# XuanchenLi/Topo4D

Measured on AMD Instinct MI355X. Metric: rasterizer fwd+bwd views/sec, higher is better.
Workload: dtype f32; 1 GPU; C2: 24 views x 512x512, P=30000 vertex-bound Gaussians, precomputed RGB, opacity scenario A, forward+backward, per-view gradients; frames=64, steps_per_rank=20, parallelism=frame-sharded x1, frames_per_launch=1, sync_mode=lazy (capacity learned by checked warm-up), frames_in_flight=3

## Files before the change

topo4d_amd/csrc/t4d_raster.hip:

```cpp
#include "t4d_raster_plan.h"

#include <hip/hip_runtime.h>
#include <stdint.h>
#include <stdio.h>
#include <string.h>
#include <vector>

#include "t4d_activations.h"
#include "t4d_tile_div.h"
#include "t4d_raster_visit_pad.h"

#define T4D_EXPORT extern "C" __attribute__((visibility("default")))

namespace {

#ifndef T4D_BWD_BATCH
#define T4D_BWD_BATCH 128
#endif
constexpr int kBwdBatch = T4D_BWD_BATCH;
constexpr int kRankSortMax = 512;
constexpr int kHist = 1024;
constexpr int kBuckets = 24;
constexpr int kGP = T4D_GRAD_PAIR_FLOATS;
constexpr int kSnapFloats = 6;

thread_local char g_err[512] = "";

enum KernelId { K_PREPROCESS = 0, K_SCAN_TILES, K_SCATTER, K_SORT_TILES, K_RENDER_FWD, K_RENDER_BWD, K_PREPROCESS_BWD,
                K_SORT_LONG, K_FWD_LONG, K_RENDER_BWD_LONG, K_COUNT };
const char *const kKernelNames[K_COUNT] = { "k_preprocess", "k_scan_tiles", "k_scatter", "k_sort_tiles", "k_render_fwd",
                                            "k_render_bwd", "k_preprocess_bwd", "k_sort_long", "k_fwd_long", "k_render_bwd_long" };
struct ProfRec { int id; hipEvent_t a, b; };
bool g_prof_on = false;
std::vector<ProfRec> g_prof;

struct Layout {
    size_t status, view_total, view_cursor, tile_count, bucket_fill, slot_tab, zero_end;
    size_t snap, live;
    size_t tile_off, chunk_sum, order, items, xy, depth, conic_opacity, rgb, clamped, pair_off, pair_rank, keys, sort_tmp, final_T, n_contrib, total;
};

struct DevStatus {
    uint32_t overflow;
    uint32_t max_pairs;
    unsigned long long total_pairs;
    uint32_t max_tile_pairs;
    uint32_t grid_sync;
    uint32_t live_segments;
};

inline size_t align_up(size_t x, size_t a = 256) { return (x + a - 1) / a * a; }

Layout make_layout(const T4DProblem &p)
{
    Layout L;
    const size_t V = (size_t)p.n_views, P = (size_t)p.P;
    const size_t T = (size_t)tile_dims(p.W, p.H).T;
    const size_t HW = (size_t)p.H * p.W;
    const size_t cap = (size_t)p.pair_capacity;
    size_t o = 0;
    L.status = o;        o = align_up(o + sizeof(DevStatus));
    L.view_total = o;    o = align_up(o + V * 4);
    L.view_cursor = o;   o = align_up(o + V * kCursorSegs * 4);
    L.tile_count = o;    o = align_up(o + V * T * 4);
    L.bucket_fill = o;   o = align_up(o + kBuckets * 4);
    const size_t slots = seg_mode(p) != 0 ? V * seg_slots_per_view(p, T) : 0;
    L.slot_tab = o;      o = align_up(o + slots * 16);
    L.zero_end = o;
    L.snap = o;          o = align_up(o + slots * kSnapFloats * kBlock * 4);
    L.live = o;          o = align_up(o + (seg_mode(p) == 2 ? slots * 4 : 0));
    L.tile_off = o;      o = align_up(o + V * T * 4);
    L.chunk_sum = o;     o = align_up(o + V * ((T + kScanChunk - 1) / kScanChunk) * 4);
    L.order = o;         o = align_up(o + (size_t)kBuckets * V * T * 4);
    L.items = o;         o = align_up(o + V * T * 16);
    L.xy = o;            o = align_up(o + V * P * 8);
    L.depth = o;         o = align_up(o + V * P * 4);
    L.conic_opacity = o; o = align_up(o + V * P * 16);
    L.rgb = o;           o = align_up(o + (p.sh_coeffs > 0 ? V * P * 12 : 0));
    L.clamped = o;       o = align_up(o + (p.sh_coeffs > 0 ? V * P : 0));
    L.pair_off = o;      o = align_up(o + V * P * 4);
    L.pair_rank = o;     o = align_up(o + V * cap * 4);
    L.keys = o;          o = align_up(o + V * cap * 8);
    L.sort_tmp = o;      o = align_up(o + V * cap * 8);
    L.final_T = o;       o = align_up(o + V * HW * 4);
    L.n_contrib = o;     o = align_up(o + V * HW * 4);
    L.total = o;
    return L;
}

struct KP {
    int V, P, H, W, gx, gy, T, deg, M;
    float scale_modifier;
    uint32_t cap;
    uint32_t nseg, seg_cap;
    uint32_t seg_shift;
    const float *views, *means3D, *opacities, *scales, *rotations, *cov3D_precomp, *colors_precomp, *shs;
    DevStatus *status;
    uint32_t *view_total, *view_cursor, *tile_count, *bucket_fill, *tile_off, *chunk_sum, *order, *pair_off, *pair_rank;
    int n_chunks;
    int long_bins_elsewhere;
    int raw_params;
    uint4 *items;
    float2 *xy;
    float *depth;
    float4 *conic_opacity;
    float *rgb;
    uint8_t *clamped;
    unsigned long long *keys, *sort_tmp;
    float *cut_r2;
    float *final_T;
    uint32_t *n_contrib;
    float *out_color, *out_depth, *out_alpha;
    int32_t *radii;
    const float *dL_dcolor, *dL_ddepth, *dL_dalpha;
    float *grad_pair;
    float *dL_dmeans3D, *dL_dmeans2D, *dL_dcolors, *dL_dshs, *dL_dopacities, *dL_dscales, *dL_drotations, *dL_dcov3D;
    float *tile_dot;
    float *cotangent_dot;
    uint32_t tile_blocks;
    uint32_t fill_blocks;
    uint32_t fill_vec;
    uint4 *slot_tab;
    float *snap;
    uint32_t slots_per_view;
    uint32_t fused_sort;
    unsigned long long *host_status;
    uint32_t seg_min_pairs;
    uint32_t *live;
    uint32_t slots_by_offset;
    uint32_t views_per_set;
    T4DDiv div_gx;
    T4DDiv div_gy;
    T4DDiv div_spans;
    T4DDiv div_blocks;
    uint32_t div_blocks_ok;
    uint32_t div_ok;
};

typedef const __attribute__((address_space(4))) KP *kp_kernarg_p;
__device__ __forceinline__ kp_kernarg_p kernarg_kp()
{
    kp_kernarg_p p = (kp_kernarg_p)__builtin_amdgcn_kernarg_segment_ptr();
    asm volatile("" : "+s"(p));
    return p;
}

__device__ __forceinline__ float ndc2pix(float v, int S)
{
#pragma clang fp contract(off)
    return ((v + 1.0f) * S - 1.0f) * 0.5f;
}

__device__ __forceinline__ void tile_rect(float px, float py, int r, int gx, int gy, int &x0, int &y0, int &x1, int &y1)
{
    x0 = min(gx, max(0, (int)((px - r) / T4D_TILE_X)));
    y0 = min(gy, max(0, (int)((py - r) / T4D_TILE_Y)));
    x1 = min(gx, max(0, (int)((px + r + T4D_TILE_X - 1) / T4D_TILE_X)));
    y1 = min(gy, max(0, (int)((py + r + T4D_TILE_Y - 1) / T4D_TILE_Y)));
}

typedef const __attribute__((address_space(4))) float *const_float_p;
struct ViewRecord {
    float view[16], proj[16], campos[3], bg[3], tanx, tany;
};
__device__ __forceinline__ ViewRecord load_view_record(const float *views, const int v)
{
    const_float_p p = (const_float_p)(views + (size_t)v * T4D_VIEW_FLOATS);
    ViewRecord r;
#pragma unroll
    for (int i = 0; i < 16; i++) { r.view[i] = p[i]; r.proj[i] = p[16 + i]; }
#pragma unroll
    for (int i = 0; i < 3; i++) { r.campos[i] = p[32 + i]; r.bg[i] = p[35 + i]; }
    r.tanx = p[38]; r.tany = p[39];
    return r;
}

__device__ __forceinline__ size_t param_row0(const KP &kp, const int v)
{
    return kp.views_per_set ? (size_t)((uint32_t)v / kp.views_per_set) * (size_t)kp.P : (size_t)0;
}

__device__ __forceinline__ uint32_t seg_slot0(const KP &kp, const uint32_t off, const uint32_t tile)
{
    static_assert((kSegLongMin & (kSegLongMin - 1)) == 0, "a shift");
    return (off >> kp.seg_shift) + (kp.slots_by_offset ? off / (uint32_t)kSegLongMin : tile);
}

__device__ __forceinline__ uint32_t wave_incl_scan(uint32_t v)
{
    const int lane = threadIdx.x & 63;
#pragma unroll
    for (int d = 1; d < 64; d <<= 1) {
        uint32_t o = __shfl_up(v, d, 64);
        if (lane >= d) v += o;
    }
    return v;
}

template <int CTRL, int ROW_MASK = 0xf, int BANK_MASK = 0xf>
__device__ __forceinline__ float dpp0(float v)
{
    return __int_as_float(__builtin_amdgcn_update_dpp(0, __float_as_int(v), CTRL, ROW_MASK, BANK_MASK, false));
}

__device__ __forceinline__ float wave_sum_to_lane63(float v)
{
    v += dpp0<0xB1>(v);
    v += dpp0<0x4E>(v);
    v += dpp0<0x141>(v);
    v += dpp0<0x140>(v);
    v += dpp0<0x142, 0xA>(v);
    v += dpp0<0x143, 0xC>(v);
    return v;
}

__device__ __forceinline__ void quat_rot(const float4 q, float R[9])
{
#pragma clang fp contract(off)
    const float r = q.x, x = q.y, y = q.z, z = q.w;
    R[0] = 1.f - 2.f * (y * y + z * z); R[1] = 2.f * (x * y - r * z);       R[2] = 2.f * (x * z + r * y);
    R[3] = 2.f * (x * y + r * z);       R[4] = 1.f - 2.f * (x * x + z * z); R[5] = 2.f * (y * z - r * x);
    R[6] = 2.f * (x * z - r * y);       R[7] = 2.f * (y * z + r * x);       R[8] = 1.f - 2.f * (x * x + y * y);
}

__device__ __forceinline__ void cov3d_from_scale_rot(const float *scale, float mod, const float4 q, float cov[6])
{
#pragma clang fp contract(off)
    float R[9], M[9];
    quat_rot(q, R);
    const float s[3] = { mod * scale[0], mod * scale[1], mod * scale[2] };
#pragma unroll
    for (int i = 0; i < 3; i++)
#pragma unroll
        for (int k = 0; k < 3; k++) M[i * 3 + k] = R[i * 3 + k] * s[k];
    cov[0] = M[0] * M[0] + M[1] * M[1] + M[2] * M[2];
    cov[1] = M[0] * M[3] + M[1] * M[4] + M[2] * M[5];
    cov[2] = M[0] * M[6] + M[1] * M[7] + M[2] * M[8];
    cov[3] = M[3] * M[3] + M[4] * M[4] + M[5] * M[5];
    cov[4] = M[3] * M[6] + M[4] * M[7] + M[5] * M[8];
    cov[5] = M[6] * M[6] + M[7] * M[7] + M[8] * M[8];
}

__device__ __forceinline__ void ewa_rows(const float *mean, const float *view, float fx, float fy, float tanx, float tany,
                                         float T0[3], float T1[3], float t[3], bool &inx, bool &iny)
{
#pragma clang fp contract(off)
    t[0] = view[0] * mean[0] + view[4] * mean[1] + view[8] * mean[2] + view[12];
    t[1] = view[1] * mean[0] + view[5] * mean[1] + view[9] * mean[2] + view[13];
    t[2] = view[2] * mean[0] + view[6] * mean[1] + view[10] * mean[2] + view[14];
    const float limx = T4D_FRUSTUM_CLAMP * tanx, limy = T4D_FRUSTUM_CLAMP * tany;
    const float txtz = t[0] / t[2], tytz = t[1] / t[2];
    inx = !(txtz < -limx || txtz > limx);
    iny = !(tytz < -limy || tytz > limy);
    t[0] = fminf(limx, fmaxf(-limx, txtz)) * t[2];
    t[1] = fminf(limy, fmaxf(-limy, tytz)) * t[2];
    const float J00 = fx / t[2], J02 = -(fx * t[0]) / (t[2] * t[2]);
    const float J11 = fy / t[2], J12 = -(fy * t[1]) / (t[2] * t[2]);
#pragma unroll
    for (int j = 0; j < 3; j++) {
        T0[j] = J00 * view[j * 4 + 0] + J02 * view[j * 4 + 2];
        T1[j] = J11 * view[j * 4 + 1] + J12 * view[j * 4 + 2];
    }
}

__device__ __forceinline__ void sym3_mul(const float c[6], const float v[3], float o[3])
{
#pragma clang fp contract(off)
    o[0] = c[0] * v[0] + c[1] * v[1] + c[2] * v[2];
    o[1] = c[1] * v[0] + c[3] * v[1] + c[4] * v[2];
    o[2] = c[2] * v[0] + c[4] * v[1] + c[5] * v[2];
}

__device__ __forceinline__ void sh_basis(int deg, const float d[3], float b[16])
{
#pragma clang fp contract(off)
    const float x = d[0], y = d[1], z = d[2];
    b[0] = T4D_SH_C0;
    if (deg > 0) {
        b[1] = -T4D_SH_C1 * y; b[2] = T4D_SH_C1 * z; b[3] = -T4D_SH_C1 * x;
        if (deg > 1) {
// ... 169 lines not shown
    kp.n_contrib = reinterpret_cast<uint32_t *>(st + L.n_contrib);
    kp.slot_tab = reinterpret_cast<uint4 *>(st + L.slot_tab);
    kp.snap = reinterpret_cast<float *>(st + L.snap);
    kp.live = reinterpret_cast<uint32_t *>(st + L.live);
    kp.div_ok = (t4d_div_make((uint32_t)kp.gx, (uint64_t)kp.T, kp.div_gx) &&
                 t4d_div_make((uint32_t)kp.gy, (uint64_t)kp.V * (uint64_t)kp.gy, kp.div_gy) &&
                 t4d_div_make(empty_spans(kp.T), (uint64_t)kp.V * empty_spans(kp.T), kp.div_spans)) ? 1u : 0u;
    return kp.div_ok != 0u;
}

void to_status(const DevStatus &hs, T4DStatus &out)
{
    out.max_pairs_per_view = hs.max_pairs;
    out.total_pairs = (int64_t)hs.total_pairs;
    out.overflow = (int32_t)hs.overflow;
    out.max_tile_pairs = (int32_t)min(hs.max_tile_pairs, 0x7fffffffu);
}

int device_cus()
{
    static int cus = 0;
    if (cus == 0) {
        int dev = 0, n = 0;
        if (hipGetDevice(&dev) != hipSuccess || hipDeviceGetAttribute(&n, hipDeviceAttributeMultiprocessorCount, dev) != hipSuccess || n <= 0)
            n = 256;
        cus = n;
    }
    return cus;
}

}

T4D_EXPORT uint32_t t4d_abi_version(void) { return T4D_ABI_VERSION; }
T4D_EXPORT const char *t4d_last_error(void) { return g_err; }

T4D_EXPORT size_t t4d_state_bytes(const T4DProblem *prob)
{
    if (check_problem(prob) != T4D_OK) return 0;
    return make_layout(*prob).total;
}

size_t grad_pair_bytes(const T4DProblem &p) { return align_up((size_t)p.n_views * (size_t)p.pair_capacity * kGP * sizeof(float)); }
size_t tile_dot_bytes(const T4DProblem &p, size_t n_tiles) { return align_up((size_t)p.n_views * n_tiles * 4 * sizeof(float)); }

T4D_EXPORT size_t t4d_backward_scratch_bytes(const T4DProblem *prob)
{
    if (check_problem(prob) != T4D_OK) return 0;
    const size_t n_tiles = (size_t)tile_dims(prob->W, prob->H).T;
    return grad_pair_bytes(*prob) + tile_dot_bytes(*prob, n_tiles) +
           (prob->sh_coeffs > 0 ? align_up((size_t)prob->n_views * (size_t)prob->P * 3 * sizeof(float)) : 0);
}

T4D_EXPORT int t4d_debug_state_layout(const T4DProblem *prob, int has_sh, uint64_t *offsets, int n)
{
    int rc = check_problem(prob);
    if (rc != T4D_OK) return rc;
    if (!offsets || n < T4D_DEBUG_LAYOUT_FIELDS) return fail(T4D_ERR_ARG, "offsets must hold T4D_DEBUG_LAYOUT_FIELDS entries");
    T4DProblem p = *prob;
    if (!has_sh) p.sh_coeffs = 0;
    const Layout L = make_layout(p);
    const size_t f[T4D_DEBUG_LAYOUT_FIELDS] = { L.status, L.view_total, L.view_cursor, L.tile_count, L.bucket_fill, L.tile_off,
                                                L.xy, L.depth, L.conic_opacity, L.rgb, L.clamped, L.pair_off, L.keys,
                                                L.final_T, L.n_contrib, L.total };
    for (int i = 0; i < T4D_DEBUG_LAYOUT_FIELDS; i++) offsets[i] = (uint64_t)f[i];
    return T4D_OK;
}

static unsigned front_small_resident_blocks()
{
    static int cached_dev = -1;
    static unsigned cached = 0;
    int dev = 0;
    if (hipGetDevice(&dev) != hipSuccess) { (void)hipGetLastError(); return 0; }
    if (dev != cached_dev) {
        int per_cu = 0, cus = 0;
        if (hipOccupancyMaxActiveBlocksPerMultiprocessor(&per_cu, k_front_small, kBlock, 0) != hipSuccess ||
            hipDeviceGetAttribute(&cus, hipDeviceAttributeMultiprocessorCount, dev) != hipSuccess || per_cu < 1 || cus < 1) {
            (void)hipGetLastError();
            per_cu = 0; cus = 0;
        }
        cached = (unsigned)per_cu * (unsigned)cus;
        cached_dev = dev;
    }
    return cached;
}

typedef void (*render_kernel_t)(const KP);
#define T4D_LAUNCH(kernel, grid, block, params) hipLaunchKernelGGL(kernel, dim3(grid), dim3(block), 0, stream, params)

static render_kernel_t render_fwd_kernel(const FwdBuild b)
{
    switch (build_key(b)) {
    case build_key(FwdBuild{ false, kFwdBatch, 0, true, true }):    return k_render_fwd<false, kFwdBatch, 0, true, true>;
    case build_key(FwdBuild{ true, kBlock, kSegOne, true, false }): return k_render_fwd<true, kBlock, kSegOne, true>;
    case build_key(FwdBuild{ true, kBlock, kSeg, true, false }):    return k_render_fwd<true, kBlock, kSeg, true>;
    case build_key(FwdBuild{ true, kBlock, 0, true, false }):       return k_render_fwd<true, kBlock, 0, true>;
    case build_key(FwdBuild{ false, kBlock, kSegOne, true, false }): return k_render_fwd<false, kBlock, kSegOne, true>;
    case build_key(FwdBuild{ false, kBlock, kSeg, true, false }):   return k_render_fwd<false, kBlock, kSeg, true>;
    case build_key(FwdBuild{ false, kFwdBatch, 0, true, false }):   return k_render_fwd<false, kFwdBatch, 0, true>;
    case build_key(FwdBuild{ false, kFwdBatch, 0, false, false }):  return k_render_fwd<false, kFwdBatch, 0, false>;
    default: return nullptr;
    }
}

static render_kernel_t render_bwd_kernel(const BwdBuild b)
{
    switch (build_key(b)) {
    case build_key(BwdBuild{ true, false, 0, true }):          return k_render_bwd<true, false, 0, true>;
    case build_key(BwdBuild{ false, false, 0, true }):         return k_render_bwd<false, false, 0, true>;
    case build_key(BwdBuild{ true, false, kSeg, true }):       return k_render_bwd<true, false, kSeg, true>;
    case build_key(BwdBuild{ false, false, kSeg, true }):      return k_render_bwd<false, false, kSeg, true>;
    case build_key(BwdBuild{ true, false, kSegOne, false }):   return k_render_bwd<true, false, kSegOne>;
    case build_key(BwdBuild{ false, false, kSegOne, false }):  return k_render_bwd<false, false, kSegOne>;
    case build_key(BwdBuild{ true, false, kSeg, false }):      return k_render_bwd<true, false, kSeg>;
    case build_key(BwdBuild{ false, false, kSeg, false }):     return k_render_bwd<false, false, kSeg>;
    case build_key(BwdBuild{ true, true, 0, false }):          return k_render_bwd<true, true, 0>;
    case build_key(BwdBuild{ false, true, 0, false }):         return k_render_bwd<false, true, 0>;
    case build_key(BwdBuild{ true, false, 0, false }):         return k_render_bwd<true, false, 0>;
    case build_key(BwdBuild{ false, false, 0, false }):        return k_render_bwd<false, false, 0>;
    default: return nullptr;
    }
}

T4D_EXPORT int t4d_rasterize_forward(const T4DProblem *prob, const T4DForwardIO *io, T4DStatus *status, void *hip_stream)
{
    int rc = check_problem(prob);
    if (rc != T4D_OK) return rc;
    if (!io || !io->views || !io->means3D || !io->opacities || !io->out_color || !io->out_depth || !io->out_alpha ||
        !io->out_radii || !io->state)
        return fail(T4D_ERR_ARG, "null required pointer in T4DForwardIO");
    KP kp;
    memset(&kp, 0, sizeof(kp));
    if ((rc = take_inputs(kp, *io)) != T4D_OK) return rc;
    if (io->shs && prob->sh_coeffs < 1) return fail(T4D_ERR_ARG, "shs given but sh_coeffs == 0");
    T4DProblem p = *prob;
    if (!io->shs) p.sh_coeffs = 0;
    const Layout L = make_layout(p);
    if (io->state_bytes < L.total) return fail(T4D_ERR_STATE_SIZE, "state buffer smaller than t4d_state_bytes()");

    const Overrides ov = read_overrides();
    const DeviceFacts dev = { device_cus(), front_small_candidate(p, ov) ? front_small_resident_blocks() : 0u };
    const bool planes_aligned16 = (((uintptr_t)io->out_color | (uintptr_t)io->out_depth | (uintptr_t)io->out_alpha) & 15u) == 0;
    const ForwardPlan plan = plan_forward(p, dev, ov, planes_aligned16);
    const render_kernel_t render = render_fwd_kernel(plan.render);
    if (!render) return fail(T4D_ERR_ARG, "internal: the plan asks for a k_render_fwd build that does not exist");

    hipStream_t stream = (hipStream_t)hip_stream;
    const bool debug = (p.flags & T4D_FLAG_DEBUG_SYNC) != 0;
    const bool checked = debug || (p.flags & T4D_FLAG_CHECKED) != 0;
    char *st = (char *)io->state;
    if (!fill_common(kp, p, plan.regime, L, st)) return fail(T4D_ERR_ARG, "no exact multiplier for this tile grid");
    kp.out_color = io->out_color; kp.out_depth = io->out_depth; kp.out_alpha = io->out_alpha; kp.radii = io->out_radii;
    kp.fused_sort = plan.fused_sort;
    kp.tile_blocks = plan.tile_blocks; kp.fill_blocks = plan.fill_blocks; kp.fill_vec = plan.fill_vec;
    const uint32_t render_grid = kp.tile_blocks + kp.fill_blocks;
    const uint64_t top = (uint64_t)render_grid * kp.fill_blocks;
    kp.div_blocks_ok = (top < (1ull << 32) && t4d_div_make(render_grid, top + 1u, kp.div_blocks)) ? 1u : 0u;
    if (plan.status_by_kernel && status) {
        void *dptr = nullptr;
        if (hipHostGetDevicePointer(&dptr, (void *)status, 0) == hipSuccess && dptr != nullptr) kp.host_status = (unsigned long long *)dptr;
        else (void)hipGetLastError();
    }

    T4D_HIP(hipMemsetAsync(st, 0, L.zero_end, stream));
    {
        ProfScope ps_(stream, K_PREPROCESS);
        if (plan.front == FrontEnd::Fused) T4D_LAUNCH(k_front_small, plan.preprocess_grid, kBlock, kp);
        else T4D_LAUNCH(k_preprocess, plan.preprocess_grid, kBlock, kp);
    }
    T4D_LAUNCH_CHECK("k_preprocess", debug);
    if (plan.front == FrontEnd::SmallView) {
        ProfScope ps_(stream, K_SCATTER);
        T4D_LAUNCH(k_scan_scatter_small, plan.small_grid, kBlock, kp);
    } else if (plan.front == FrontEnd::General) {
        ProfScope ps_(stream, K_SCAN_TILES);
        if (plan.chunk_sums) T4D_LAUNCH(k_tile_chunk_sums, dim3(plan.scan_grid_x, plan.scan_grid_y), kScanChunk, kp);
        T4D_LAUNCH(k_scan_tiles, dim3(plan.scan_grid_x, plan.scan_grid_y), kScanChunk, kp);
    }
    T4D_LAUNCH_CHECK("k_scan_tiles", debug);
    if (checked) {
        DevStatus hs;
        T4D_HIP(hipMemcpyAsync(&hs, st + L.status, sizeof(hs), hipMemcpyDeviceToHost, stream));
        T4D_HIP(hipStreamSynchronize(stream));
        if (status) to_status(hs, *status);
        if (hs.overflow) return fail(T4D_ERR_PAIR_OVERFLOW, "pair_capacity too small for this scene");
    } else if ((p.flags & T4D_FLAG_ASYNC_STATUS) && status && !kp.host_status) {
        T4D_HIP(hipMemcpyAsync((void *)status, st + L.status, 16, hipMemcpyDeviceToHost, stream));
    }
    if (plan.front == FrontEnd::General) {
        ProfScope ps_(stream, K_SCATTER);
        T4D_LAUNCH(k_scatter, plan.scatter_grid, kBlock, kp);
    }
    T4D_LAUNCH_CHECK("k_scatter", debug);
    if (plan.sorter != Sorter::Fused) {
        ProfScope ps_(stream, K_SORT_TILES);
        if (plan.sorter == Sorter::Block1024) T4D_LAUNCH(k_sort_tiles<kLongBlock>, plan.sort_grid, kLongBlock, kp);
        else T4D_LAUNCH(k_sort_tiles<kBlock>, plan.sort_grid, kBlock, kp);
    }
    T4D_LAUNCH_CHECK("k_sort_tiles", debug);
    if (plan.long_bins) {
        ProfScope ps_(stream, K_SORT_LONG);
        T4D_LAUNCH(k_sort_long_chunks, plan.long_bins_grid, kLongBlock, kp);
        T4D_LAUNCH(k_merge_long, plan.long_bins_grid, kLongBlock, kp);
    }
    T4D_LAUNCH_CHECK("k_sort_long", debug);
    {
        ProfScope ps_(stream, K_RENDER_FWD);
        T4D_LAUNCH(render, render_grid, kBlock, kp);
    }
    T4D_LAUNCH_CHECK("k_render_fwd", debug);
    if (plan.long_fwd) {
        ProfScope ps_(stream, K_FWD_LONG);
        KP kl = kp;
        kl.tile_blocks = plan.long_seg_grid;
        T4D_LAUNCH(k_fwd_long_seg<false>, plan.long_seg_grid, kBlock, kl);
        T4D_LAUNCH_CHECK("k_fwd_long_seg", debug);
        T4D_LAUNCH(k_fwd_long_prefix, plan.long_prefix_grid, kBlock, kl);
        T4D_LAUNCH_CHECK("k_fwd_long_prefix", debug);
        T4D_LAUNCH(k_fwd_long_seg<true>, plan.long_seg_grid, kBlock, kl);
        T4D_LAUNCH_CHECK("k_fwd_long_seg", debug);
    }
    return T4D_OK;
}

T4D_EXPORT int t4d_rasterize_backward(const T4DProblem *prob, const T4DBackwardIO *io, void *hip_stream)
{
    int rc = check_problem(prob);
    if (rc != T4D_OK) return rc;
    if (!io || !io->views || !io->means3D || !io->opacities || !io->radii || !io->state || !io->dL_dcolor ||
        !io->dL_dmeans3D || !io->dL_dmeans2D || !io->dL_dopacities || !io->scratch)
        return fail(T4D_ERR_ARG, "null required pointer in T4DBackwardIO");
    KP kp;
    memset(&kp, 0, sizeof(kp));
    if ((rc = take_inputs(kp, *io)) != T4D_OK) return rc;
    if (io->shs ? !io->dL_dshs : !io->dL_dcolors) return fail(T4D_ERR_ARG, "missing colour gradient output");
    if (io->cov3D_precomp ? !io->dL_dcov3D : (!io->dL_dscales || !io->dL_drotations))
        return fail(T4D_ERR_ARG, "missing covariance gradient output");
    T4DProblem p = *prob;
    if (!io->shs) p.sh_coeffs = 0;
    const Layout L = make_layout(p);
    if (io->state_bytes < L.total) return fail(T4D_ERR_STATE_SIZE, "state buffer smaller than t4d_state_bytes()");
    if (io->scratch_bytes < t4d_backward_scratch_bytes(&p))
        return fail(T4D_ERR_STATE_SIZE, "scratch smaller than t4d_backward_scratch_bytes()");

    const Overrides ov = read_overrides();
    const DeviceFacts dev = { device_cus(), 0u };
    const BackwardPlan plan = plan_backward(p, dev, ov, io->dL_ddepth || io->dL_dalpha, io->cotangent_dot != nullptr, io->shs != nullptr);
    render_kernel_t render[2] = { nullptr, nullptr };
    for (int i = 0; i < plan.n_render; i++)
        if (!(render[i] = render_bwd_kernel(plan.render[i].build)))
            return fail(T4D_ERR_ARG, "internal: the plan asks for a k_render_bwd build that does not exist");

    hipStream_t stream = (hipStream_t)hip_stream;
    const bool debug = (p.flags & T4D_FLAG_DEBUG_SYNC) != 0;
    if (!fill_common(kp, p, plan.regime, L, (char *)io->state)) return fail(T4D_ERR_ARG, "no exact multiplier for this tile grid");
    kp.radii = const_cast<int32_t *>(io->radii);
    kp.dL_dcolor = io->dL_dcolor; kp.dL_ddepth = io->dL_ddepth; kp.dL_dalpha = io->dL_dalpha;
    kp.grad_pair = (float *)io->scratch;
    if (io->cotangent_dot) {
        kp.tile_dot = (float *)((char *)io->scratch + grad_pair_bytes(p));
        kp.cotangent_dot = io->cotangent_dot;
    }
    kp.dL_dmeans3D = io->dL_dmeans3D; kp.dL_dmeans2D = io->dL_dmeans2D; kp.dL_dcolors = io->dL_dcolors;
    kp.dL_dshs = io->dL_dshs; kp.dL_dopacities = io->dL_dopacities; kp.dL_dscales = io->dL_dscales;
    kp.dL_drotations = io->dL_drotations; kp.dL_dcov3D = io->dL_dcov3D;

    for (int i = 0; i < plan.n_render; i++) {
        {
            ProfScope ps_(stream, i == 0 ? K_RENDER_BWD : K_RENDER_BWD_LONG);
            kp.tile_blocks = plan.render[i].tile_blocks;
            T4D_LAUNCH(render[i], plan.render[i].grid, kBlock, kp);
        }
        T4D_LAUNCH_CHECK("k_render_bwd", debug);
    }
    {
        ProfScope ps_(stream, K_PREPROCESS_BWD);
        if (kp.shs)
            kp.dL_dcolors = (float *)((char *)io->scratch + grad_pair_bytes(p) + tile_dot_bytes(p, (size_t)kp.T));
        T4D_LAUNCH(k_preprocess_bwd, plan.gaussian_grid, kBlock, kp);
        if (plan.sh == ShBackward::Degree3x16) T4D_LAUNCH(k_sh_bwd16, plan.sh_grid, kBlock, kp);
        else if (plan.sh == ShBackward::General) T4D_LAUNCH(k_sh_bwd, plan.sh_grid, kBlock, kp);
    }
    T4D_LAUNCH_CHECK("k_preprocess_bwd", debug);
    return T4D_OK;
}

T4D_EXPORT int t4d_profile_begin(void)
{
    for (auto &r : g_prof) { (void)hipEventDestroy(r.a); (void)hipEventDestroy(r.b); }
    g_prof.clear();
    g_prof_on = true;
    return T4D_OK;
}

T4D_EXPORT int t4d_profile_end(T4DKernelTime *out, int max_entries, int *n_entries)
{
    g_prof_on = false;
    if (!out || !n_entries || max_entries < K_COUNT) return fail(T4D_ERR_ARG, "need room for every kernel");
    for (int k = 0; k < K_COUNT; k++) {
        out[k].name = kKernelNames[k];
        out[k].total_ms = 0.0;
        out[k].launches = 0;
    }
    for (auto &r : g_prof) {
        T4D_HIP(hipEventSynchronize(r.b));
        float ms = 0.f;
// ... 49 lines not shown
```

topo4d_amd/csrc/t4d_raster_plan.h:

```cpp
#pragma once
#include <stdint.h>
#include <stdlib.h>
#include <unistd.h>

#include <algorithm>

#include "../../include/t4d_config.h"
#include "../../include/topo4d_raster.h"

#ifndef T4D_HD
#if defined(__HIPCC__) || defined(__CUDACC__)
#define T4D_HD __host__ __device__
#else
#define T4D_HD
#endif
#endif

constexpr int kBlock = 256;
#ifndef T4D_FWD_BATCH
#define T4D_FWD_BATCH 192
#endif
constexpr int kFwdBatch = T4D_FWD_BATCH;
constexpr int kSortLdsCap = 2048;
constexpr int kLongBlock = 1024;
constexpr int kScanChunk = 1024;
constexpr int kCursorSegs = 64;
#ifndef T4D_SEG
#define T4D_SEG 128
#endif
constexpr int kSeg = T4D_SEG;
constexpr int kSegOne = 64;
constexpr int kSegMaxTiles = 8192;
#ifndef T4D_SEG_LONG_MIN
#define T4D_SEG_LONG_MIN 2048
#endif
constexpr int kSegLongMin = T4D_SEG_LONG_MIN;
static_assert((kSegLongMin & (kSegLongMin - 1)) == 0, "k_fwd_long_prefix stops at the first work item of a shorter length CLASS (powers of two)");
static_assert(kSegOne == 64 && kSeg == 128, "seg_shift assumes segment lengths of 64 and 128");
constexpr int kSmallTiles = 4 * kBlock;
constexpr int kEmptySpan = 64;
#ifndef T4D_SHB_VIEWS
#define T4D_SHB_VIEWS 8
#endif
constexpr int kMaxGridPerCu = 96;

struct TileDims { int gx, gy; int64_t T; };
inline TileDims tile_dims(const int W, const int H)
{
    TileDims d;
    d.gx = (W + T4D_TILE_X - 1) / T4D_TILE_X;
    d.gy = (H + T4D_TILE_Y - 1) / T4D_TILE_Y;
    d.T = (int64_t)d.gx * (int64_t)d.gy;
    return d;
}

inline int seg_mode(const T4DProblem &p)
{
    if ((long long)p.n_views * tile_dims(p.W, p.H).T <= kSegMaxTiles) return 1;
    return p.n_views == 1 ? 2 : 0;
}
inline int seg_positions(const T4DProblem &p) { return (p.n_views == 1 && seg_mode(p) == 1) ? kSegOne : kSeg; }
inline size_t seg_slots_per_view(const T4DProblem &p, size_t T)
{
    if (seg_mode(p) == 2) return (size_t)p.pair_capacity / (size_t)kSeg + (size_t)p.pair_capacity / (size_t)kSegLongMin + 2;
    return (size_t)p.pair_capacity / (size_t)seg_positions(p) + T + 1;
}

T4D_HD inline unsigned gaussian_grid(const int P, const int V) { return (unsigned)((((P + kBlock - 1) / kBlock + 7) / 8) * 8 * V); }

struct Regime {
    int gx, gy, T;
    int seg_mode;
    uint32_t slots_per_view;
    uint32_t seg_shift;
    uint32_t slots_by_offset;
    uint32_t seg_min_pairs;
    uint32_t views_per_set;
    uint32_t nseg, seg_cap;
    int n_chunks;
    int long_bins_elsewhere;
    int segn;
};
inline Regime regime_of(const T4DProblem &p)
{
    Regime r;
    const TileDims d = tile_dims(p.W, p.H);
    r.gx = d.gx; r.gy = d.gy; r.T = (int)d.T;
    r.seg_mode = seg_mode(p);
    r.slots_per_view = r.seg_mode != 0 ? (uint32_t)seg_slots_per_view(p, (size_t)r.T) : 0u;
    r.seg_shift = seg_positions(p) == 64 ? 6u : 7u;
    r.slots_by_offset = r.seg_mode == 2 ? 1u : 0u;
    r.seg_min_pairs = r.seg_mode == 2 ? ((p.flags & T4D_FLAG_NO_LONG_BINS) ? 0xffffffffu : (uint32_t)kSegLongMin) : 0u;
    r.views_per_set = (p.views_per_param_set != 0u && p.views_per_param_set < (uint32_t)p.n_views) ? p.views_per_param_set : 0u;
    const uint32_t n_wg = (uint32_t)((p.P + kBlock - 1) / kBlock);
    r.nseg = 1;
    while (r.nseg < (uint32_t)kCursorSegs && n_wg >= 16u * r.nseg) r.nseg <<= 1;
    r.seg_cap = (uint32_t)p.pair_capacity / r.nseg;
    r.n_chunks = (r.T + kScanChunk - 1) / kScanChunk;
    r.long_bins_elsewhere = (p.flags & T4D_FLAG_NO_LONG_BINS) ? 0 : 1;
    r.segn = (r.slots_per_view != 0u && r.seg_min_pairs != 0xffffffffu) ? seg_positions(p) : 0;
    return r;
}

struct Overrides {
    bool has_latency_tiles = false, has_fwd_latency_tiles = false;
    int latency_tiles = 0;
    int fwd_latency_tiles = 0;
    int tile_div = 0;
    bool no_segments = false;
    bool no_long_fwd = false;
    bool no_fused_sort = false;
    bool sort_256 = false;
    bool no_front_fusion = false;
    bool status_by_copy = false;
    bool no_prune = false;
    bool no_small_view = false;
    bool fill_scalar = false;
    bool sh_bwd_plain = false;
};
inline Overrides read_overrides()
{
    Overrides o;
    bool any = false;
    for (char **e = environ; e && *e && !any; e++) any = (*e)[0] == 'T' && (*e)[1] == '4' && (*e)[2] == 'D' && (*e)[3] == '_';
    if (!any) return o;
    if (const char *e = getenv("T4D_LATENCY_TILES")) { o.has_latency_tiles = true; o.latency_tiles = atoi(e); }
    if (const char *e = getenv("T4D_FWD_LATENCY_TILES")) { o.has_fwd_latency_tiles = true; o.fwd_latency_tiles = atoi(e); }
    if (const char *e = getenv("T4D_TILE_DIV")) o.tile_div = atoi(e);
    o.no_segments = getenv("T4D_NO_SEGMENTS") != nullptr;
    o.no_long_fwd = getenv("T4D_NO_LONG_FWD") != nullptr;
    o.no_fused_sort = getenv("T4D_NO_FUSED_SORT") != nullptr;
    o.sort_256 = getenv("T4D_SORT_256") != nullptr;
    o.no_front_fusion = getenv("T4D_NO_FRONT_FUSION") != nullptr;
    o.status_by_copy = getenv("T4D_STATUS_BY_COPY") != nullptr;
    o.no_prune = getenv("T4D_NO_PRUNE") != nullptr;
    o.no_small_view = getenv("T4D_NO_SMALL_VIEW") != nullptr;
    o.fill_scalar = getenv("T4D_FILL_SCALAR") != nullptr;
    o.sh_bwd_plain = getenv("T4D_SH_BWD_PLAIN") != nullptr;
    return o;
}

struct DeviceFacts {
    int cus;
    unsigned front_resident_blocks;
};

inline int tile_grid(const int n_tiles, const int per_cu, const int div, const DeviceFacts &dev, const Overrides &ov)
{
    if (ov.tile_div > 0) return std::max(std::min(n_tiles, dev.cus * per_cu), (n_tiles + ov.tile_div - 1) / ov.tile_div);
    return std::max(std::min(n_tiles, dev.cus * per_cu), std::min((n_tiles + div - 1) / div, dev.cus * kMaxGridPerCu));
}

inline bool latency_launch(const int n_tiles, const DeviceFacts &dev, const Overrides &ov)
{
    return n_tiles <= (ov.has_latency_tiles ? ov.latency_tiles : 4 * dev.cus);
}
inline bool latency_launch_fwd(const int n_tiles, const uint32_t flags, const DeviceFacts &dev, const Overrides &ov)
{
    if (ov.has_fwd_latency_tiles) return n_tiles <= ov.fwd_latency_tiles;
    if (ov.has_latency_tiles) return n_tiles <= ov.latency_tiles;
    return n_tiles <= ((flags & T4D_FLAG_LONG_LISTS) ? 24 : 12) * dev.cus;
}

inline bool small_view(const T4DProblem &p, const Overrides &ov)
{
    return p.n_views == 1 && tile_dims(p.W, p.H).T <= kSmallTiles && !ov.no_small_view;
}
inline bool front_small_candidate(const T4DProblem &p, const Overrides &ov)
{
    return small_view(p, ov) && gaussian_grid(p.P, 1) + 1u <= 128u && !ov.no_front_fusion;
}

enum class FrontEnd {
    Fused,
    SmallView,
    General
};
enum class Sorter { Fused , Block1024 , Block256  };
struct FwdBuild { bool lat; int fb; int segn; bool prune; bool long_elsewhere; };
constexpr uint32_t build_key(const FwdBuild b)
{
    return (uint32_t)b.lat | (uint32_t)b.prune << 1 | (uint32_t)b.long_elsewhere << 2 | (uint32_t)b.fb << 4 | (uint32_t)b.segn << 16;
}

struct ForwardPlan {
    Regime regime;
    FrontEnd front;
    unsigned preprocess_grid;
    unsigned small_grid;
    bool chunk_sums;
    unsigned scan_grid_x, scan_grid_y, scatter_grid;
    bool status_by_kernel;
    Sorter sorter;
    unsigned sort_grid;
    bool long_bins;
    unsigned long_bins_grid;
    FwdBuild render;
    uint32_t tile_blocks, fill_blocks, fill_vec;
    bool long_fwd;
    unsigned long_seg_grid, long_prefix_grid;
    uint32_t fused_sort;
};

inline ForwardPlan plan_forward(const T4DProblem &p, const DeviceFacts &dev, const Overrides &ov, const bool planes_aligned16)
{
    ForwardPlan f = {};
    const Regime &r = f.regime = regime_of(p);
    const int n_tiles = r.T * p.n_views;
    const bool checked = (p.flags & (T4D_FLAG_DEBUG_SYNC | T4D_FLAG_CHECKED)) != 0;

    f.front = !small_view(p, ov) ? FrontEnd::General
            : (front_small_candidate(p, ov) && gaussian_grid(p.P, 1) + 1u <= dev.front_resident_blocks) ? FrontEnd::Fused : FrontEnd::SmallView;
    f.preprocess_grid = f.front == FrontEnd::Fused ? gaussian_grid(p.P, 1) + 1u : gaussian_grid(p.P, p.n_views);
    f.small_grid = gaussian_grid(p.P, 1) + 1u;
    f.chunk_sums = r.n_chunks > 1;
    f.scan_grid_x = (unsigned)r.n_chunks; f.scan_grid_y = (unsigned)p.n_views;
    f.scatter_grid = gaussian_grid(p.P, p.n_views) + (unsigned)(((size_t)r.T * p.n_views + kBlock - 1) / kBlock);
    f.status_by_kernel = !checked && (p.flags & T4D_FLAG_ASYNC_STATUS) != 0 && small_view(p, ov) && !ov.status_by_copy;

    const bool lat = latency_launch_fwd(n_tiles, p.flags, dev, ov);
    f.long_fwd = r.seg_mode == 2 && r.segn != 0 && !lat && !ov.no_long_fwd;
    f.fused_sort = (!ov.no_fused_sort && (f.long_fwd || (lat && (p.flags & T4D_FLAG_SHORT_BINS) != 0))) ? 1u : 0u;
    if (f.fused_sort) { f.sorter = Sorter::Fused; f.sort_grid = 0; }
    else if (r.seg_mode == 1 && (p.flags & T4D_FLAG_SHORT_BINS) == 0 && !ov.sort_256) { f.sorter = Sorter::Block1024; f.sort_grid = (unsigned)std::min(n_tiles, 4 * dev.cus); }
    else { f.sorter = Sorter::Block256; f.sort_grid = (unsigned)tile_grid(n_tiles, 5, 2, dev, ov); }
    f.long_bins = r.long_bins_elsewhere != 0;
    f.long_bins_grid = (unsigned)std::min(n_tiles, 2 * dev.cus);

    f.tile_blocks = (uint32_t)(lat ? n_tiles : tile_grid(n_tiles, 6, 2, dev, ov));
    f.fill_blocks = (uint32_t)(r.gy * p.n_views);
    f.fill_vec = (p.W % 4 == 0 && planes_aligned16 && !ov.fill_scalar) ? 1u : 0u;
    if (f.long_fwd) f.render = { false, kFwdBatch, 0, true, true };
    else if (lat || r.segn != 0) f.render = { lat, kBlock, r.segn, true, false };
    else f.render = { false, kFwdBatch, 0, r.long_bins_elsewhere != 0 && !ov.no_prune, false };
    f.long_seg_grid = std::min(r.slots_per_view, (uint32_t)(8 * dev.cus));
    f.long_prefix_grid = std::min((uint32_t)r.T, (uint32_t)(4 * dev.cus));
    return f;
}

struct BwdBuild { bool da, lat; int segn; bool long_elsewhere; };
constexpr uint32_t build_key(const BwdBuild b)
{
    return (uint32_t)b.da | (uint32_t)b.lat << 1 | (uint32_t)b.long_elsewhere << 2 | (uint32_t)b.segn << 16;
}
struct BwdLaunch { BwdBuild build; uint32_t tile_blocks; unsigned grid; };
enum class ShBackward { None, Degree3x16 , General  };

struct BackwardPlan {
    Regime regime;
    int n_render;
    BwdLaunch render[2];
    unsigned gaussian_grid;
    ShBackward sh;
    unsigned sh_grid;
};

inline BackwardPlan plan_backward(const T4DProblem &p, const DeviceFacts &dev, const Overrides &ov, const bool da,
                                  const bool wants_tile_dot, const bool has_shs)
{
    BackwardPlan b = {};
    const Regime &r = b.regime = regime_of(p);
    const int n_tiles = r.T * p.n_views;
    const bool lat = latency_launch(n_tiles, dev, ov);
    const bool seg = r.seg_mode == 1 && !ov.no_segments;
    const bool seg_long = r.seg_mode == 2 && r.segn != 0 && !ov.no_segments;
    const uint32_t tile_blocks = seg ? (uint32_t)p.n_views * r.slots_per_view : (uint32_t)(lat ? n_tiles : tile_grid(n_tiles, 4, 2, dev, ov));
    const unsigned grid = tile_blocks + (wants_tile_dot ? (uint32_t)p.n_views * (uint32_t)((r.T + kEmptySpan - 1) / kEmptySpan) : 0u);
    b.n_render = 1;
    if (seg_long) {
        b.n_render = 2;
        b.render[0] = { { da, false, 0, true }, tile_blocks, grid };
        const uint32_t walkers = std::min(r.slots_per_view, (uint32_t)(8 * dev.cus));
        b.render[1] = { { da, false, kSeg, true }, walkers, walkers };
    } else if (seg) {
        b.render[0] = { { da, false, r.segn, false }, tile_blocks, grid };
    } else {
        b.render[0] = { { da, lat, 0, false }, tile_blocks, grid };
    }
    b.gaussian_grid = gaussian_grid(p.P, p.n_views) + (wants_tile_dot ? (unsigned)p.n_views : 0u);
    if (!has_shs) { b.sh = ShBackward::None; b.sh_grid = 0; }
    else if (p.sh_coeffs == 16 && p.sh_degree == 3 && !ov.sh_bwd_plain && (r.views_per_set == 0u || r.views_per_set % T4D_SHB_VIEWS == 0u)) {
        b.sh = ShBackward::Degree3x16;
        b.sh_grid = gaussian_grid(p.P, (p.n_views + T4D_SHB_VIEWS - 1) / T4D_SHB_VIEWS);
    } else {
        b.sh = ShBackward::General;
        b.sh_grid = gaussian_grid(p.P, p.n_views);
    }
    return b;
}
```

topo4d_amd/csrc/t4d_raster_sort.h:

```cpp
template <int J>
__device__ __forceinline__ uint32_t lane_xor(const uint32_t v)
{
    if (J == 1) return (uint32_t)__builtin_amdgcn_update_dpp(0, (int)v, 0xB1, 0xf, 0xf, true);
    if (J == 2) return (uint32_t)__builtin_amdgcn_update_dpp(0, (int)v, 0x4E, 0xf, 0xf, true);
    if (J == 4) {
        const int t = __builtin_amdgcn_update_dpp(0, (int)v, 0x104, 0xf, 0x5, true);
        return (uint32_t)__builtin_amdgcn_update_dpp(t, (int)v, 0x114, 0xf, 0xA, true);
    }
    if (J == 8) return (uint32_t)__builtin_amdgcn_update_dpp(0, (int)v, 0x128, 0xf, 0xf, true);
    return (uint32_t)__shfl_xor((int)v, J, 64);
}

template <int K, int J>
__device__ __forceinline__ void bitonic_step(unsigned long long &key, const int lane)
{
    const unsigned long long other = ((unsigned long long)lane_xor<J>((uint32_t)(key >> 32)) << 32) | lane_xor<J>((uint32_t)key);
    const bool keep_min = ((lane & J) == 0) == ((lane & K) == 0);
    key = ((other < key) == keep_min) ? other : key;
    if constexpr (J > 1) bitonic_step<K, J / 2>(key, lane);
}

__device__ __forceinline__ void wave_sort64(unsigned long long &key, const int lane)
{
    bitonic_step<2, 1>(key, lane);
    bitonic_step<4, 2>(key, lane);
    bitonic_step<8, 4>(key, lane);
    bitonic_step<16, 8>(key, lane);
    bitonic_step<32, 16>(key, lane);
    bitonic_step<64, 32>(key, lane);
}

__device__ __forceinline__ uint32_t run_lower_bound(const unsigned long long *run, const unsigned long long key)
{
    uint32_t pos = 0;
#pragma unroll
    for (int st = 32; st > 0; st >>= 1)
        if (run[pos + st - 1] < key) pos += st;
    return pos + (run[pos] < key ? 1u : 0u);
}

__device__ __forceinline__ uint32_t lower_bound_global(const unsigned long long *run, const uint32_t len, const uint32_t cap2,
                                                       const unsigned long long key)
{
    uint32_t pos = 0;
    for (uint32_t st = cap2 >> 1; st > 0; st >>= 1)
        if (pos + st <= len && run[pos + st - 1] < key) pos += st;
    return pos + ((pos < len && run[pos] < key) ? 1u : 0u);
}

template <int BLOCK, int CAP, int PRE = 0>
__device__ __forceinline__ void sort_chunk_lds(unsigned long long *keys, const uint32_t n, unsigned long long *s_keys,
                                               const int tid, const int wave, const int lane, unsigned long long *dst = nullptr)
{
    if (dst == nullptr) dst = keys;
    constexpr int kPer = CAP / BLOCK;
    const uint32_t runs = (n + 63u) >> 6, N = runs << 6;
    for (uint32_t r = (uint32_t)wave; r < runs; r += BLOCK / 64) {
        const uint32_t i = (r << 6) + (uint32_t)lane;
        unsigned long long k0 = i < n ? keys[i] : ~0ull;
        if (PRE == 0) wave_sort64(k0, lane);
        s_keys[i] = k0;
    }
    __syncthreads();
    for (uint32_t w = PRE != 0 ? (uint32_t)PRE : 64u; w < N; w <<= 1) {
        unsigned long long kk[kPer];
        uint32_t np[kPer];
#pragma unroll
        for (int e = 0; e < kPer; e++) {
            const uint32_t p = (uint32_t)tid + e * BLOCK;
            if (p < N) {
                kk[e] = s_keys[p];
                const uint32_t run = p / w, sbase = (run ^ 1u) * w;
                const uint32_t slen = sbase < N ? min(w, N - sbase) : 0u;
                const unsigned long long *sib = s_keys + sbase;
                uint32_t pos = 0;
                for (uint32_t st = w >> 1; st > 0; st >>= 1)
                    if (pos + st <= slen && sib[pos + st - 1] < kk[e]) pos += st;
                if (pos < slen && sib[pos] < kk[e]) pos++;
                np[e] = (run & ~1u) * w + (p & (w - 1u)) + pos;
            }
        }
        __syncthreads();
#pragma unroll
        for (int e = 0; e < kPer; e++)
            if ((uint32_t)tid + e * BLOCK < N) s_keys[np[e]] = kk[e];
        __syncthreads();
    }
    for (uint32_t i = tid; i < n; i += BLOCK) dst[i] = s_keys[i];
    __syncthreads();
}

template <int BLOCK, int CAP, int PRE = 0>
__device__ __forceinline__ void sort_bin_chunked(unsigned long long *keys, unsigned long long *tmp, const uint32_t n,
                                                 unsigned long long *s_keys, const int tid, const int wave, const int lane)
{
    for (uint32_t c = 0; c < n; c += CAP) sort_chunk_lds<BLOCK, CAP, PRE>(keys + c, min((uint32_t)CAP, n - c), s_keys, tid, wave, lane);
    unsigned long long *src = keys, *dst = tmp;
    for (uint32_t w = CAP; w < n; w <<= 1) {
        __threadfence_block();
        __syncthreads();
        for (uint32_t i0 = (uint32_t)tid * 4u; i0 < n; i0 += BLOCK * 4u) {
            unsigned long long kk[4];
            uint32_t slot[4];
#pragma unroll
            for (int e = 0; e < 4; e++) kk[e] = i0 + e < n ? src[i0 + e] : ~0ull;
#pragma unroll
            for (int e = 0; e < 4; e++) {
                const uint32_t i = i0 + e, run = i / w, sbase = (run ^ 1u) * w;
                const uint32_t slen = sbase < n ? min(w, n - sbase) : 0u;
                slot[e] = (run & ~1u) * w + (i & (w - 1u)) + lower_bound_global(src + sbase, slen, w, kk[e]);
            }
#pragma unroll
            for (int e = 0; e < 4; e++)
                if (i0 + e < n) dst[slot[e]] = kk[e];
        }
        unsigned long long *t2 = src; src = dst; dst = t2;
    }
    if (src != keys) {
        __threadfence_block();
        __syncthreads();
        for (uint32_t i = tid; i < n; i += BLOCK) keys[i] = src[i];
    }
}

template <bool KEEP, int BLOCK>
__device__ __forceinline__ void sort_one_bin(const KP &kp, const int v, const uint32_t off, const uint32_t n, unsigned long long *s_keys,
                                             const int tid, const int wave, const int lane)
{
    unsigned long long *keys = kp.keys + (size_t)v * kp.cap + off;
    if (n <= (uint32_t)kRankSortMax) {
        constexpr int kWaves = BLOCK / 64;
        constexpr int kPer = kRankSortMax / BLOCK > 0 ? kRankSortMax / BLOCK : 1;
        const uint32_t runs = (n + 63u) >> 6;
        unsigned long long mine[kPer];
        uint32_t ranks[kPer];
#pragma unroll
        for (int e = 0; e < kPer; e++) {
            const uint32_t i = (uint32_t)tid + e * BLOCK;
            if ((uint32_t)(wave + kWaves * e) < runs) {
                mine[e] = i < n ? keys[i] : ~0ull;
                wave_sort64(mine[e], lane);
                s_keys[i] = mine[e];
            }
        }
        __syncthreads();
#pragma unroll
        for (int e = 0; e < kPer; e++) {
            const uint32_t own = (uint32_t)(wave + kWaves * e);
            ranks[e] = 0xffffffffu;
            if (own < runs) {
                uint32_t rank = (uint32_t)lane;
#pragma unroll
                for (uint32_t r = 0; r < (uint32_t)(kRankSortMax / 64); r++)
                    if (r < runs && r != own) rank += run_lower_bound(s_keys + ((r % kWaves) * 64u + (r / kWaves) * BLOCK), mine[e]);
                if (mine[e] != ~0ull) { keys[rank] = mine[e]; ranks[e] = rank; }
            }
        }
        if (KEEP) {
            __syncthreads();
#pragma unroll
            for (int e = 0; e < kPer; e++)
                if (ranks[e] != 0xffffffffu) s_keys[ranks[e]] = mine[e];
        }
    } else if (n <= (uint32_t)kSortLdsCap) {
        sort_chunk_lds<BLOCK, kSortLdsCap>(keys, n, s_keys, tid, wave, lane);
    } else if (!kp.long_bins_elsewhere) {
        sort_bin_chunked<BLOCK, kSortLdsCap>(keys, kp.sort_tmp + (size_t)v * kp.cap + off, n, s_keys, tid, wave, lane);
    }
}

template <int BLOCK>
__global__ __launch_bounds__(BLOCK) void k_sort_tiles(const KP kp)
{
    constexpr int kWaves = BLOCK / 64;
    __shared__ unsigned long long s_keys[kSortLdsCap];
    const int tid = threadIdx.x, wave = tid >> 6, lane = tid & 63;
    constexpr int kClass63 = (kBuckets - 2) - 5, kClass1 = kBuckets - 2;
    uint32_t n_big = 0, n_small = 0;
#pragma unroll
    for (int k = 0; k < kBuckets - 1; k++) {
        const uint32_t f = kp.bucket_fill[k];
        if (k < kClass63) n_big += f;
        else if (k < kClass1) n_small += f;
    }
    const uint32_t n_units = n_big + ((n_small + kWaves - 1u) / kWaves);
    for (uint32_t unit = blockIdx.x; unit < n_units; unit += gridDim.x) {
        if (unit >= n_big) {
            const uint32_t item = n_big + (uint32_t)kWaves * (unit - n_big) + (uint32_t)wave;
            if (item < n_big + n_small) {
                const uint4 it = kp.items[item];
                const uint32_t n = it.z;
                unsigned long long *keys = kp.keys + (size_t)(it.x >> 20) * kp.cap + it.y;
                unsigned long long k0 = (uint32_t)lane < n ? keys[lane] : ~0ull;
                wave_sort64(k0, lane);
                if ((uint32_t)lane < n) keys[lane] = k0;
            }
            continue;
        }
        const uint4 it = kp.items[unit];
        sort_one_bin<false, BLOCK>(kp, (int)(it.x >> 20), it.y, it.z, s_keys, tid, wave, lane);
        __syncthreads();
    }
}

constexpr int kLongScan = 1024;

template <typename F>
__device__ __forceinline__ void for_each_long_chunk(const KP &kp, uint32_t *s_first, uint32_t *s_wsum, F &&unit)
{
    static_assert(kLongScan == kLongBlock, "one work item per thread and round");
    const int tid = threadIdx.x, wave = tid >> 6, lane = tid & 63;
    const uint32_t n_items = (uint32_t)(kp.V * kp.T);
    uint32_t units_before = 0;
    for (uint32_t base = 0; base < n_items; base += kLongScan) {
        const uint32_t i = base + (uint32_t)tid;
        const uint32_t n_i = i < n_items ? kp.items[i].z : 0u;
        const uint32_t c_i = n_i > (uint32_t)kSortLdsCap ? (n_i + (uint32_t)kSortLdsCap - 1u) / (uint32_t)kSortLdsCap : 0u;
        const uint32_t incl = wave_incl_scan(c_i);
        if (lane == 63) s_wsum[wave] = incl;
        const bool more = __syncthreads_or(tid == kLongScan - 1 && n_i >= (uint32_t)kSortLdsCap);
        uint32_t woff = 0, total = 0;
#pragma unroll
        for (int w = 0; w < kLongBlock / 64; w++) {
            const uint32_t x = s_wsum[w];
            if (w < wave) woff += x;
            total += x;
        }
        s_first[tid] = woff + incl - c_i;
        if (tid == 0) s_first[kLongScan] = total;
        __syncthreads();
        for (uint32_t u = blockIdx.x + ((units_before + gridDim.x - 1u - blockIdx.x) / gridDim.x) * gridDim.x; u < units_before + total; u += gridDim.x) {
            const uint32_t lu = u - units_before;
            uint32_t pos = 0;
#pragma unroll
            for (uint32_t st = kLongScan >> 1; st > 0; st >>= 1)
                if (s_first[pos + st] <= lu) pos += st;
            unit(kp.items[base + pos], (lu - s_first[pos]) * (uint32_t)kSortLdsCap);
        }
        units_before += total;
        if (!more) break;
        __syncthreads();
    }
}

__global__ __launch_bounds__(kLongBlock) void k_sort_long_chunks(const KP kp)
{
    __shared__ unsigned long long s_keys[kSortLdsCap];
    __shared__ uint32_t s_first[kLongScan + 1];
    __shared__ uint32_t s_wsum[kLongBlock / 64];
    const int tid = threadIdx.x, wave = tid >> 6, lane = tid & 63;
    for_each_long_chunk(kp, s_first, s_wsum, [&](const uint4 it, const uint32_t c) {
        const size_t base = (size_t)(it.x >> 20) * kp.cap + it.y + c;
        sort_chunk_lds<kLongBlock, kSortLdsCap>(kp.keys + base, min((uint32_t)kSortLdsCap, it.z - c), s_keys, tid, wave, lane, kp.sort_tmp + base);
    });
}

__global__ __launch_bounds__(kLongBlock) void k_merge_long(const KP kp)
{
    constexpr int kGroup = 4;
    __shared__ unsigned long long s_sib[kGroup * kSortLdsCap];
    __shared__ uint32_t s_first[kLongScan + 1];
    __shared__ uint32_t s_wsum[kLongBlock / 64];
    constexpr int kPer = kSortLdsCap / kLongBlock;
    static_assert(kPer == 2, "two keys per thread, their searches in lock-step");
    const int tid = threadIdx.x;
    for_each_long_chunk(kp, s_first, s_wsum, [&](const uint4 it, const uint32_t c) {
        const uint32_t n = it.z;
        const size_t base = (size_t)(it.x >> 20) * kp.cap + it.y;
        const unsigned long long *src = kp.sort_tmp + base;
        unsigned long long *dst = kp.keys + base;
        const uint32_t len = min((uint32_t)kSortLdsCap, n - c);
        unsigned long long key[kPer];
        uint32_t rank[kPer];
#pragma unroll
        for (int e = 0; e < kPer; e++) {
            const uint32_t i = (uint32_t)tid + (uint32_t)e * kLongBlock;
            key[e] = i < len ? src[c + i] : ~0ull;
            rank[e] = i;
        }
        for (uint32_t s0 = 0; s0 < n; s0 += (uint32_t)(kGroup * kSortLdsCap)) {
            const uint32_t glen = min((uint32_t)(kGroup * kSortLdsCap), n - s0);
            __syncthreads();
            for (uint32_t i = (uint32_t)tid * 2u; i < glen; i += 2u * kLongBlock) {
                const unsigned long long a = src[s0 + i];
                const unsigned long long b = i + 1u < glen ? src[s0 + i + 1u] : ~0ull;
                s_sib[i] = a; s_sib[i + 1u] = b;
            }
            __syncthreads();
            uint32_t lb[kPer][kGroup], sl[kGroup];
#pragma unroll
            for (int j = 0; j < kGroup; j++) {
                const uint32_t s = s0 + (uint32_t)j * (uint32_t)kSortLdsCap;
                sl[j] = (s < n && s != c) ? min((uint32_t)kSortLdsCap, n - s) : 0u;
#pragma unroll
                for (int e = 0; e < kPer; e++) lb[e][j] = 0u;
            }
            for (uint32_t st = (uint32_t)kSortLdsCap >> 1; st > 0; st >>= 1) {
#pragma unroll
                for (int j = 0; j < kGroup; j++)
#pragma unroll
                    for (int e = 0; e < kPer; e++) {
                        const uint32_t p = lb[e][j] + st;
                        if (p <= sl[j] && s_sib[j * kSortLdsCap + p - 1u] < key[e]) lb[e][j] = p;
                    }
            }
#pragma unroll
            for (int j = 0; j < kGroup; j++)
#pragma unroll
                for (int e = 0; e < kPer; e++)
                    rank[e] += lb[e][j] + ((lb[e][j] < sl[j] && s_sib[j * kSortLdsCap + lb[e][j]] < key[e]) ? 1u : 0u);
        }
#pragma unroll
        for (int e = 0; e < kPer; e++)
            if ((uint32_t)tid + (uint32_t)e * kLongBlock < len) dst[rank[e]] = key[e];
    });
}
```

Baseline: 61210 views/s.

## Sort mid-sized tile bins with per-wave register bitonic networks

```diff
diff --git a/topo4d_amd/csrc/t4d_raster.hip b/topo4d_amd/csrc/t4d_raster.hip
--- a/topo4d_amd/csrc/t4d_raster.hip
+++ b/topo4d_amd/csrc/t4d_raster.hip
@@ -1,4 +1,5 @@
 #include "t4d_raster_plan.h"
+#include "t4d_raster_sort_net.h"
 
 #include <hip/hip_runtime.h>
 #include <stdint.h>
@@ -126,6 +127,7 @@
     uint32_t fused_sort;
     unsigned long long *host_status;
     uint32_t seg_min_pairs;
+    uint32_t wave_bins;
     uint32_t *live;
     uint32_t slots_by_offset;
     uint32_t views_per_set;
@@ -601,6 +603,7 @@
     if (!fill_common(kp, p, plan.regime, L, st)) return fail(T4D_ERR_ARG, "no exact multiplier for this tile grid");
     kp.out_color = io->out_color; kp.out_depth = io->out_depth; kp.out_alpha = io->out_alpha; kp.radii = io->out_radii;
     kp.fused_sort = plan.fused_sort;
+    kp.wave_bins = plan.wave_bins ? 1u : 0u;
     kp.tile_blocks = plan.tile_blocks; kp.fill_blocks = plan.fill_blocks; kp.fill_vec = plan.fill_vec;
     const uint32_t render_grid = kp.tile_blocks + kp.fill_blocks;
     const uint64_t top = (uint64_t)render_grid * kp.fill_blocks;
diff --git a/topo4d_amd/csrc/t4d_raster_plan.h b/topo4d_amd/csrc/t4d_raster_plan.h
--- a/topo4d_amd/csrc/t4d_raster_plan.h
+++ b/topo4d_amd/csrc/t4d_raster_plan.h
@@ -117,6 +117,7 @@
     bool no_small_view = false;
     bool fill_scalar = false;
     bool sh_bwd_plain = false;
+    bool no_wave_sort = false;
 };
 inline Overrides read_overrides()
 {
@@ -137,6 +138,7 @@
     o.no_small_view = getenv("T4D_NO_SMALL_VIEW") != nullptr;
     o.fill_scalar = getenv("T4D_FILL_SCALAR") != nullptr;
     o.sh_bwd_plain = getenv("T4D_SH_BWD_PLAIN") != nullptr;
+    o.no_wave_sort = getenv("T4D_NO_WAVE_SORT") != nullptr;
     return o;
 }
 
@@ -193,6 +195,7 @@
     bool status_by_kernel;
     Sorter sorter;
     unsigned sort_grid;
+    bool wave_bins;
     bool long_bins;
     unsigned long_bins_grid;
     FwdBuild render;
@@ -224,6 +227,7 @@
     if (f.fused_sort) { f.sorter = Sorter::Fused; f.sort_grid = 0; }
     else if (r.seg_mode == 1 && (p.flags & T4D_FLAG_SHORT_BINS) == 0 && !ov.sort_256) { f.sorter = Sorter::Block1024; f.sort_grid = (unsigned)std::min(n_tiles, 4 * dev.cus); }
     else { f.sorter = Sorter::Block256; f.sort_grid = (unsigned)tile_grid(n_tiles, 5, 2, dev, ov); }
+    f.wave_bins = f.sorter == Sorter::Block256 && !ov.no_wave_sort;
     f.long_bins = r.long_bins_elsewhere != 0;
     f.long_bins_grid = (unsigned)std::min(n_tiles, 2 * dev.cus);
 
diff --git a/topo4d_amd/csrc/t4d_raster_sort.h b/topo4d_amd/csrc/t4d_raster_sort.h
--- a/topo4d_amd/csrc/t4d_raster_sort.h
+++ b/topo4d_amd/csrc/t4d_raster_sort.h
@@ -169,6 +169,56 @@
     }
 }
 
+template <int K, int S>
+__device__ __forceinline__ void net_stages(unsigned long long (&key)[K], const int lane)
+{
+    namespace sn = t4d_sort_net;
+    constexpr sn::Stage st = sn::stage_at(S);
+    if constexpr (sn::in_lane(st, K)) {
+#pragma unroll
+        for (int e = 0; e < K; e++) {
+            if ((e & st.j) != 0) continue;
+            const unsigned long long a = key[e], b = key[e | st.j];
+            const bool swap = (b < a) == sn::keeps_min(st, K, lane, e);
+            key[e] = swap ? b : a;
+            key[e | st.j] = swap ? a : b;
+        }
+    } else {
+        constexpr int J = sn::lane_distance(st, K);
+        const bool keep_min = sn::keeps_min(st, K, lane, 0);
+#pragma unroll
+        for (int e = 0; e < K; e++) {
+            const unsigned long long other = ((unsigned long long)lane_xor<J>((uint32_t)(key[e] >> 32)) << 32) | lane_xor<J>((uint32_t)key[e]);
+            key[e] = ((other < key[e]) == keep_min) ? other : key[e];
+        }
+    }
+    if constexpr (S + 1 < sn::stage_count(sn::elements(K))) net_stages<K, S + 1>(key, lane);
+}
+
+template <int K>
+__device__ __forceinline__ void sort_bin_wave(unsigned long long *keys, const uint32_t n, const int lane)
+{
+    unsigned long long key[K];
+    const uint32_t i0 = (uint32_t)lane * K;
+#pragma unroll
+    for (int e = 0; e < K; e++) key[e] = i0 + e < n ? keys[i0 + e] : ~0ull;
+    if constexpr (K == 1) wave_sort64(key[0], lane);
+    else net_stages<K, 0>(key, lane);
+#pragma unroll
+    for (int e = 0; e < K; e++)
+        if (i0 + e < n) keys[i0 + e] = key[e];
+}
+
+__device__ __noinline__ void sort_bin_wave_long(unsigned long long *keys, const uint32_t n, const int lane)
+{
+    if (n <= 128u) sort_bin_wave<2>(keys, n, lane);
+    else if (n <= 256u) sort_bin_wave<4>(keys, n, lane);
+    else sort_bin_wave<8>(keys, n, lane);
+}
+
+constexpr int kClassWaveTop = (kBuckets - 2) - 8;
+static_assert((2 << 8) == 64 * t4d_sort_net::kMaxKeysPerLane, "the classes up to kClassWaveTop fit the largest network");
+
 template <int BLOCK>
 __global__ __launch_bounds__(BLOCK) void k_sort_tiles(const KP kp)
 {
@@ -177,10 +227,13 @@
     const int tid = threadIdx.x, wave = tid >> 6, lane = tid & 63;
     constexpr int kClass63 = (kBuckets - 2) - 5, kClass1 = kBuckets - 2;
     uint32_t n_big = 0, n_small = 0;
+    bool wave_bins = false;
+    if constexpr (BLOCK == kBlock) wave_bins = kp.wave_bins != 0u;
 #pragma unroll
     for (int k = 0; k < kBuckets - 1; k++) {
         const uint32_t f = kp.bucket_fill[k];
-        if (k < kClass63) n_big += f;
+        if (k < kClassWaveTop) n_big += f;
+        else if (k < kClass63) { if (wave_bins) n_small += f; else n_big += f; }
         else if (k < kClass1) n_small += f;
     }
     const uint32_t n_units = n_big + ((n_small + kWaves - 1u) / kWaves);
@@ -191,6 +244,12 @@
                 const uint4 it = kp.items[item];
                 const uint32_t n = it.z;
                 unsigned long long *keys = kp.keys + (size_t)(it.x >> 20) * kp.cap + it.y;
+                if constexpr (BLOCK == kBlock) {
+                    if (n > 64u) {
+                        sort_bin_wave_long(keys, n, lane);
+                        continue;
+                    }
+                }
                 unsigned long long k0 = (uint32_t)lane < n ? keys[lane] : ~0ull;
                 wave_sort64(k0, lane);
                 if ((uint32_t)lane < n) keys[lane] = k0;
diff --git a/topo4d_amd/csrc/t4d_raster_sort_net.h b/topo4d_amd/csrc/t4d_raster_sort_net.h
--- /dev/null
+++ b/topo4d_amd/csrc/t4d_raster_sort_net.h
@@ -0,0 +1,47 @@
+#pragma once
+
+#ifndef T4D_HD
+#if defined(__HIPCC__) || defined(__CUDACC__)
+#define T4D_HD __host__ __device__
+#else
+#define T4D_HD
+#endif
+#endif
+
+namespace t4d_sort_net {
+
+constexpr int kLanes = 64;
+constexpr int kMaxKeysPerLane = 8;
+
+struct Stage { int k, j; };
+
+T4D_HD constexpr int log2i(const int n) { return n <= 1 ? 0 : 1 + log2i(n / 2); }
+T4D_HD constexpr int elements(const int K) { return kLanes * K; }
+T4D_HD constexpr int stage_count(const int N) { return log2i(N) * (log2i(N) + 1) / 2; }
+T4D_HD constexpr Stage stage_at(const int s, const int level = 1)
+{
+    return s < level ? Stage{ 1 << level, (1 << level) >> (s + 1) } : stage_at(s - level, level + 1);
+}
+T4D_HD constexpr bool in_lane(const Stage st, const int K) { return st.j < K; }
+T4D_HD constexpr int in_lane_stages(const int K, const int s = 0)
+{
+    return s >= stage_count(elements(K)) ? 0 : (in_lane(stage_at(s), K) ? 1 : 0) + in_lane_stages(K, s + 1);
+}
+T4D_HD constexpr int lane_distance(const Stage st, const int K) { return st.j / K; }
+
+T4D_HD constexpr bool bit_clear(const int K, const int lane, const int e, const int bit)
+{
+    return bit < K ? (e & bit) == 0 : (lane & (bit / K)) == 0;
+}
+T4D_HD constexpr bool keeps_min(const Stage st, const int K, const int lane, const int e)
+{
+    return bit_clear(K, lane, e, st.j) == bit_clear(K, lane, e, st.k);
+}
+
+T4D_HD constexpr int keys_per_lane(const unsigned n) { return n <= 64u ? 1 : n <= 128u ? 2 : n <= 256u ? 4 : 8; }
+
+static_assert(stage_count(64) == 21 && stage_count(512) == 45, "21 cross-lane stages, 0 / 7 / 15 / 24 in-lane ones");
+static_assert(in_lane_stages(1) == 0 && in_lane_stages(2) == 7 && in_lane_stages(4) == 15 && in_lane_stages(8) == 24, "");
+static_assert(stage_at(0).k == 2 && stage_at(0).j == 1 && stage_at(2).k == 4 && stage_at(2).j == 1 && stage_at(20).k == 64 && stage_at(20).j == 1, "");
+
+}
```

Result: faster. 62000 views/s (median of 6 runs) (+1.3%).
